# hou-yz/MVDeTr

Hardware: AMD Instinct MI355X
Metric: multiview frames/s (7-cam Wildtrack) + MSDeformAttn HBM GB/s vs roofline (higher is better)
Workload: dtype f32

## Files before the change

include/mvdetr_ops.h:

```cpp
#ifndef MVDETR_OPS_H
#define MVDETR_OPS_H

#include <stdint.h>

#ifdef __cplusplus
extern "C" {
#endif

#define MVDETR_OPS_ABI_VERSION 18

int mvdetr_ops_abi_version(void);

int mvdetr_msda_forward_f32(void *stream, const float *value, const int64_t *spatial_shapes,
                            const int64_t *level_start_index, const float *sampling_loc,
                            const float *attn_weight, int batch, int spatial_size, int num_heads,
                            int channels, int num_levels, int num_query, int num_point, float *out);
int mvdetr_msda_forward_f64(void *stream, const double *value, const int64_t *spatial_shapes,
                            const int64_t *level_start_index, const double *sampling_loc,
                            const double *attn_weight, int batch, int spatial_size, int num_heads,
                            int channels, int num_levels, int num_query, int num_point, double *out);

int mvdetr_msda_forward_f16(void *stream, const uint16_t *value, const int64_t *spatial_shapes,
                            const int64_t *level_start_index, const uint16_t *sampling_loc,
                            const uint16_t *attn_weight, int batch, int spatial_size, int num_heads, int channels,
// ... 120 lines not shown
                               const float *beta, float eps, int n, int h, int w, int channels, float *y);
int mvdetr_bn_act_f16(void *stream, const uint16_t *x, const float *mean, const float *var, const float *gamma,
                      const float *beta, float eps, const uint16_t *res, const float *res_mean, const float *res_var,
                      const float *res_gamma, const float *res_beta, float res_eps, int64_t rows, int channels, int relu,
                      uint16_t *y);
int mvdetr_bn_act_bf16(void *stream, const uint16_t *x, const float *mean, const float *var, const float *gamma,
                       const float *beta, float eps, const uint16_t *res, const float *res_mean, const float *res_var,
                       const float *res_gamma, const float *res_beta, float res_eps, int64_t rows, int channels, int relu,
                       uint16_t *y);
int mvdetr_bn_relu_maxpool_f16(void *stream, const uint16_t *x, const float *mean, const float *var, const float *gamma,
                               const float *beta, float eps, int n, int h, int w, int channels, uint16_t *y);
int mvdetr_bn_relu_maxpool_bf16(void *stream, const uint16_t *x, const float *mean, const float *var, const float *gamma,
                                const float *beta, float eps, int n, int h, int w, int channels, uint16_t *y);
const char *mvdetr_trunk_last_kernel(void);
int64_t mvdetr_trunk_launch_count(void);

int mvdetr_winograd_weights_f32(const float *w, int C, int K, float *U, void *stream);
int mvdetr_conv3x3_winograd_f32(const float *x, const float *U, float *y, int N, int H, int W, int C, int K, int dilation,
                                void *stream);
int mvdetr_conv3x3_winograd_bn_act_f32(const float *x, const float *U, float *y, int N, int H, int W, int C, int K,
                                       int dilation, const float *mean, const float *var, const float *gamma,
                                       const float *beta, float eps, const float *res, const float *res_mean,
                                       const float *res_var, const float *res_gamma, const float *res_beta, float res_eps,
                                       int relu, void *stream);
const char *mvdetr_winograd_last_kernel(void);
const char *mvdetr_winograd_last_epilogue(void);
int64_t mvdetr_winograd_launch_count(void);
int mvdetr_winograd_set_max_workgroups(int n);
int mvdetr_winograd_set_variant(int variant);
int mvdetr_winograd_last_variant(void);
int mvdetr_winograd_set_tail(int mode);
int mvdetr_winograd_last_tail_units(void);
int mvdetr_winograd_plan(int N, int H, int W, int C, int K, int dilation, int workgroups, int64_t *out);

int mvdetr_winograd_weights_dgrad_f32(const float *w, int C, int K, float *Ut, void *stream);
int mvdetr_conv3x3_winograd_wgrad_f32(const float *x, const float *gy, float *gw, int N, int H, int W, int C, int K, int dilation,
                                      void *workspace, int64_t workspace_bytes, void *stream);
int64_t mvdetr_winograd_wgrad_workspace_bytes(int N, int H, int W, int C, int K, int dilation, int workgroups);
int mvdetr_winograd_wgrad_plan(int N, int H, int W, int C, int K, int dilation, int workgroups, int64_t *out);
int mvdetr_winograd_set_wgrad_splits(int n);
int mvdetr_winograd_last_wgrad_splits(void);

const char *mvdetr_msda_last_forward_impl(void);
const char *mvdetr_msda_last_forward_kernel(void);
const char *mvdetr_msda_last_backward_route(void);

int mvdetr_msda_last_forward_resources(int *num_regs, int *scratch_bytes_per_lane, int *static_lds_bytes);

const char *mvdetr_warp_last_kernel(void);

int mvdetr_warp_release_scratch(void);

int mvdetr_msda_set_forward_impl(int impl);

int mvdetr_msda_set_backward_deterministic(int on);
int mvdetr_msda_get_backward_deterministic(void);

int mvdetr_msda_release_scratch(void);

int mvdetr_transpose_f32(void *stream, const float *src, int n, int rows, int cols, float *dst);
int mvdetr_transpose_f64(void *stream, const double *src, int n, int rows, int cols, double *dst);

int mvdetr_deform_conv2d_forward_f32(void *stream, const float *input, const float *offset, const float *weight,
                                     const float *bias, int batch, int in_channels, int in_h, int in_w, int out_channels,
                                     int kernel_h, int kernel_w, int stride_h, int stride_w, int pad_h, int pad_w, int dil_h,
                                     int dil_w, int offset_groups, int input_nhwc, float *out);
// ... 233 lines not shown
```

mvdetr_amd/_lib.py:

```python
from __future__ import annotations

import ctypes
import functools
import os
import subprocess

import torch

_HERE = os.path.dirname(os.path.abspath(__file__))
CSRC = os.path.join(_HERE, "csrc")
LIB_PATH = os.environ.get("MVDETR_OPS_LIB") or os.path.join(CSRC, "libmvdetr_ops.so")
ABI_VERSION = 18

_vp, _i = ctypes.c_void_p, ctypes.c_int
_MSDA_FWD = [_vp] * 6 + [_i] * 7 + [_vp]
_MSDA_BWD = [_vp] * 7 + [_i] * 7 + [_vp] * 3
_WARP = [_vp] * 3 + [_i] * 7 + [_vp]
_MSDA_FWD_HOST = [_vp] * 5 + [_i] * 7 + [_vp]
_MSDA_BWD_HOST = [_vp] * 6 + [_i] * 7 + [_vp] * 3
_WARP_HOST = [_vp] * 2 + [_i] * 8 + [_vp]
_MSDA_FUSED = [_vp] * 5 + [ctypes.c_int64] + [_vp] * 2 + [_i] * 10 + [_vp]
_MSDA_FUSED_HALF = [_vp] * 5 + [ctypes.c_int64, _vp] + [_i] * 7 + [_vp]
_MSDA_FUSED_LEVELS = [_vp] * 5 + [ctypes.c_int64] + [_vp] * 2 + [_i] * 12 + [_vp]
_DC_FWD = [_vp] * 5 + [_i] * 15 + [_vp]
# ... 48 lines not shown
    "mvdetr_msda_forward_fused_bf16": (_MSDA_FUSED_HALF, _i),
    "mvdetr_msda_fused_levels_supported": ([_i] * 9, _i),
    "mvdetr_msda_forward_fused_levels_f32": (_MSDA_FUSED_LEVELS, _i),
    "mvdetr_msda_fused_train_supported": ([_i] * 7, _i),
    "mvdetr_msda_forward_fused_train_f32": ([_vp] * 5 + [ctypes.c_int64, _vp] + [_i] * 7 + [_vp, _vp], _i),
    "mvdetr_msda_backward_fused_f32": ([_vp] * 6 + [ctypes.c_int64, _vp, _i, _vp, _vp] + [_i] * 6 + [_vp, _vp], _i),
    "mvdetr_msda_backward_f32": (_MSDA_BWD, _i),
    "mvdetr_msda_backward_f64": (_MSDA_BWD, _i),
    "mvdetr_add_layernorm_f32": ([_vp] * 5 + [ctypes.c_int64, _i, ctypes.c_float, _vp], _i),
    "mvdetr_add_layernorm_add_f32": ([_vp] * 6 + [ctypes.c_int64, ctypes.c_int64, _i, ctypes.c_float, _vp, _vp], _i),
    "mvdetr_add_layernorm_add_f16": ([_vp] * 6 + [ctypes.c_int64, ctypes.c_int64, _i, ctypes.c_float, _vp, _vp], _i),
    "mvdetr_add_layernorm_add_bf16": ([_vp] * 6 + [ctypes.c_int64, ctypes.c_int64, _i, ctypes.c_float, _vp, _vp], _i),
    "mvdetr_add_layernorm_last_kernel": ([], ctypes.c_char_p),
    "mvdetr_bn_act_f32": ([_vp] * 6 + [ctypes.c_float] + [_vp] * 5 + [ctypes.c_float, ctypes.c_int64, _i, _i, _vp], _i),
    "mvdetr_bn_relu_maxpool_f32": ([_vp] * 6 + [ctypes.c_float] + [_i] * 4 + [_vp], _i),
    "mvdetr_bn_act_f16": ([_vp] * 6 + [ctypes.c_float] + [_vp] * 5 + [ctypes.c_float, ctypes.c_int64, _i, _i, _vp], _i),
    "mvdetr_bn_act_bf16": ([_vp] * 6 + [ctypes.c_float] + [_vp] * 5 + [ctypes.c_float, ctypes.c_int64, _i, _i, _vp], _i),
    "mvdetr_bn_relu_maxpool_f16": ([_vp] * 6 + [ctypes.c_float] + [_i] * 4 + [_vp], _i),
    "mvdetr_bn_relu_maxpool_bf16": ([_vp] * 6 + [ctypes.c_float] + [_i] * 4 + [_vp], _i),
    "mvdetr_trunk_last_kernel": ([], ctypes.c_char_p),
    "mvdetr_trunk_launch_count": ([], ctypes.c_int64),
    "mvdetr_winograd_weights_f32": ([_vp, _i, _i, _vp, _vp], _i),
    "mvdetr_conv3x3_winograd_f32": ([_vp] * 3 + [_i] * 6 + [_vp], _i),
    "mvdetr_conv3x3_winograd_bn_act_f32": ([_vp] * 3 + [_i] * 6 + [_vp] * 4 + [ctypes.c_float] + [_vp] * 5
                                           + [ctypes.c_float, _i, _vp], _i),
    "mvdetr_winograd_last_kernel": ([], ctypes.c_char_p),
    "mvdetr_winograd_last_epilogue": ([], ctypes.c_char_p),
    "mvdetr_winograd_launch_count": ([], ctypes.c_int64),
    "mvdetr_winograd_set_max_workgroups": ([_i], _i),
    "mvdetr_winograd_set_tail": ([_i], _i),
    "mvdetr_winograd_set_variant": ([_i], _i),
    "mvdetr_winograd_last_variant": ([], _i),
    "mvdetr_winograd_last_tail_units": ([], _i),
    "mvdetr_winograd_plan": ([_i] * 7 + [_vp], _i),
    "mvdetr_winograd_weights_dgrad_f32": ([_vp, _i, _i, _vp, _vp], _i),
    "mvdetr_conv3x3_winograd_wgrad_f32": ([_vp] * 3 + [_i] * 6 + [_vp, ctypes.c_int64, _vp], _i),
    "mvdetr_winograd_wgrad_workspace_bytes": ([_i] * 7, ctypes.c_int64),
    "mvdetr_winograd_wgrad_plan": ([_i] * 7 + [_vp], _i),
    "mvdetr_winograd_set_wgrad_splits": ([_i], _i),
    "mvdetr_winograd_last_wgrad_splits": ([], _i),
    "mvdetr_warp_perspective_forward_f32": (_WARP, _i),
    "mvdetr_warp_perspective_forward_f64": (_WARP, _i),
    "mvdetr_warp_perspective_forward_f16": (_WARP, _i),
    "mvdetr_warp_perspective_forward_bf16": (_WARP, _i),
    "mvdetr_warp_perspective_backward_f32": (_WARP, _i),
    "mvdetr_warp_perspective_backward_f64": (_WARP, _i),
    "mvdetr_warp_perspective_backward_tagged_f32": ([_vp] * 3 + [_i] * 7 + [ctypes.c_uint64, _vp], _i),
    "mvdetr_warp_perspective_backward_tagged_f64": ([_vp] * 3 + [_i] * 7 + [ctypes.c_uint64, _vp], _i),
    "mvdetr_warp_backward_plan_bytes": ([_i] * 7, ctypes.c_int64),
    "mvdetr_warp_backward_plan_f32": ([_vp, _vp] + [_i] * 6 + [_vp], _i),
    "mvdetr_warp_backward_plan_f64": ([_vp, _vp] + [_i] * 6 + [_vp], _i),
    "mvdetr_warp_perspective_backward_planned_f32": ([_vp] * 4 + [_i] * 7 + [_vp], _i),
    "mvdetr_warp_perspective_backward_planned_f64": ([_vp] * 4 + [_i] * 7 + [_vp], _i),
    "mvdetr_transpose_f32": ([_vp, _vp, _i, _i, _i, _vp], _i),
    "mvdetr_transpose_f64": ([_vp, _vp, _i, _i, _i, _vp], _i),
    "mvdetr_msda_forward_host_f32": (_MSDA_FWD_HOST, _i),
    "mvdetr_msda_forward_host_f64": (_MSDA_FWD_HOST, _i),
    "mvdetr_msda_backward_host_f32": (_MSDA_BWD_HOST, _i),
    "mvdetr_msda_backward_host_f64": (_MSDA_BWD_HOST, _i),
    "mvdetr_warp_perspective_forward_host_f32": (_WARP_HOST, _i),
    "mvdetr_warp_perspective_forward_host_f64": (_WARP_HOST, _i),
    "mvdetr_warp_perspective_backward_host_f32": (_WARP_HOST, _i),
    "mvdetr_warp_perspective_backward_host_f64": (_WARP_HOST, _i),
    "mvdetr_deform_conv2d_last_kernel": ([], ctypes.c_char_p),
    "mvdetr_deform_conv2d_route_kind": ([_i] * 18, _i),
    "mvdetr_deform_conv2d_forward_f32": (_DC_FWD, _i),
# ... 140 lines not shown
```

mvdetr_amd/csrc/conv_winograd.hip:

```cpp
#include "bn_epilogue.h"
#include "common.h"
#include "conv_winograd.h"
#include "../../include/mvdetr_ops.h"

#include <atomic>
#include <type_traits>

namespace mvdetr {

std::atomic<const char *> g_winograd_last_kernel{"none"};
static std::atomic<const char *> g_winograd_last_epilogue{"none"};
std::atomic<int64_t> g_winograd_launches{0};
std::atomic<int> g_winograd_max_workgroups{0};
static std::atomic<int> g_winograd_tail{1};
static std::atomic<int> g_winograd_last_tail_units{0};
static std::atomic<int> g_winograd_variant{0};
static std::atomic<int> g_winograd_last_variant{0};

namespace wino {

constexpr int CC = 8;
constexpr int VCOLS = TILES + 8;
constexpr int VROW = VCOLS * 4;
constexpr int V_FLOATS = CC * 4 * VROW;
constexpr int U_FLOATS = 16 * CC * KB;
constexpr int BUF_FLOATS = U_FLOATS + V_FLOATS;
constexpr int TINFO_SLOTS = 4;
constexpr int LDS_BYTES = 2 * BUF_FLOATS * 4 + TINFO_SLOTS * TILES * 16;

constexpr unsigned Y_NONE = 0xFFFFFFFFu;

using f32x16 = __attribute__((ext_vector_type(16))) float;
using f32x4 = __attribute__((ext_vector_type(4))) float;

typedef __attribute__((address_space(3))) void lds_void;

struct Epilogue {
    BnVectors bn, bn2;
    const float *res;
};

template <int MODE, bool RELU>
__global__ __launch_bounds__(256) void conv3x3_winograd_f32(const float *__restrict__ x, const float *__restrict__ U,
                                                            float *__restrict__ y, const Shape s, const Epilogue ep)
{
    extern __shared__ __attribute__((aligned(16))) float lds[];
    using u32x4 = __attribute__((ext_vector_type(4))) unsigned;
    u32x4 *const tinfo = reinterpret_cast<u32x4 *>(lds + 2 * BUF_FLOATS);

    const int tid = threadIdx.x, lane = tid & 63;
// ... 461 lines not shown
        const u32x4 dsc = ti[16 * (b >> 2) + (b & 3)];
#pragma unroll
        for (int e = 0; e < 4; ++e) {
            o4[b][e] = __builtin_elementwise_add_sat(dsc[e], (unsigned)kcol * 4u);
            if (MODE >= 2) q4[b][e] = __builtin_bit_cast(float, __builtin_amdgcn_raw_buffer_load_b32(rrsrc, (int)o4[b][e], 0, 0));
        }
    }
#pragma unroll
    for (int b = 0; b < 8; ++b) {
        const int h = b >> 2, r = b & 3;
        float s0[4], s1[4];
#pragma unroll
        for (int nu = 0; nu < 4; ++nu) {
            s0[nu] = acc[nu][h][r] + acc[4 + nu][h][r] + acc[8 + nu][h][r];
            s1[nu] = acc[4 + nu][h][r] - acc[8 + nu][h][r] - acc[12 + nu][h][r];
        }
        float y00 = s0[0] + s0[1] + s0[2], y01 = s0[1] - s0[2] - s0[3];
        float y10 = s1[0] + s1[1] + s1[2], y11 = s1[1] - s1[2] - s1[3];
        if (MODE >= 1) {
            constexpr int RES = MODE - 1;
            y00 = bn_finish<RES, RELU>(bn_apply(y00, bs, bt), RES ? q4[b][0] : 0.f, bs2);
            y01 = bn_finish<RES, RELU>(bn_apply(y01, bs, bt), RES ? q4[b][1] : 0.f, bs2);
            y10 = bn_finish<RES, RELU>(bn_apply(y10, bs, bt), RES ? q4[b][2] : 0.f, bs2);
            y11 = bn_finish<RES, RELU>(bn_apply(y11, bs, bt), RES ? q4[b][3] : 0.f, bs2);
        }
        const float y4[4] = {y00, y01, y10, y11};
#pragma unroll
        for (int e = 0; e < 4; ++e)
            __builtin_amdgcn_raw_buffer_store_b32(__builtin_bit_cast(unsigned, y4[e]), yrsrc, (int)o4[b][e], 0, 0);
    }
    asm volatile("s_waitcnt vmcnt(0)" ::: "memory");
}

template <int MODE, bool RELU>
__global__ __launch_bounds__(512) void conv3x3_winograd_w16x2_f32(const float *__restrict__ x, const float *__restrict__ U,
                                                                  float *__restrict__ y, const Shape s, const Epilogue ep)
{
    extern __shared__ __attribute__((aligned(16))) float lds[];
    using u32x4 = __attribute__((ext_vector_type(4))) unsigned;
    u32x4 *const tinfo = reinterpret_cast<u32x4 *>(lds + 2 * BUF_FLOATS);

    const int tid = threadIdx.x, lane = tid & 63;
    const int wave = __builtin_amdgcn_readfirstlane(tid >> 6);
    const int C = s.C, K = s.K, d = s.d, H = s.H, W = s.W;
    const int chunks = C / CC;
    const unsigned G = gridDim.x;

    const int ltile = tid >> 3, lc = tid & 7;
    unsigned off[16];
    __amdgpu_buffer_rsrc_t xrsrc;
    __amdgpu_buffer_rsrc_t ursrc;
    struct Place { int kb, X, Y, n; };
    auto next_unit = [&](Place &p) {
        p.kb += s.gr;
        const bool carry = p.kb >= s.kblocks;
        p.kb -= carry ? s.kblocks : 0;
        tile_step(s, carry, p.X, p.Y, p.n);
        return carry;
    };
    Place sp, cpl;
    sp.kb = (int)(blockIdx.x % (unsigned)s.kblocks);
    tile_grid(s, blockIdx.x / (unsigned)s.kblocks * TILES, sp.X, sp.Y, sp.n);
    cpl = sp;
    int lX, lY, ln;
    tile_grid(s, blockIdx.x / (unsigned)s.kblocks * TILES + ltile, lX, lY, ln);
    auto enter_unit = [&](int slot) {
        const int n0 = sp.n;
        xrsrc = __builtin_amdgcn_make_buffer_rsrc(const_cast<float *>(x + (size_t)n0 * H * W * C), 0, (int)X_RANGE, 0x00020000);
        ursrc = __builtin_amdgcn_make_buffer_rsrc(const_cast<float *>(U + sp.kb * KB), 0,
                                                  (int)(((unsigned)(16 * C) * K - sp.kb * KB) * 4u), 0x00020000);
        int y0, x0;
        tile_pixel(s, lX, lY, y0, x0);
        const bool tvalid = ln < s.N;
        const unsigned pix = ((unsigned)(ln - n0) * H + y0) * W + x0;
        const unsigned base = (pix * C + lc) * 4u, cstep = (unsigned)d * C * 4u, rstep = cstep * W;
        bool oky[4], okx[4];
// ... 69 lines not shown
    f32x4 acc[16][2];
    float fa[2][2][8], fb[2][8];
    auto read_piece = [&](const float *buf, int hs, int q) {
        const int st = hs >> 1, half = hs & 1;
        if ((q & 2) == 0) {
            const int xl = q >> 2, h = q & 1;
            const f32x4 v = *reinterpret_cast<const f32x4 *>(buf + a_off + (16 * st + 2 * half + xl) * VROW + (16 * h + 4 * st) * 4);
#pragma unroll
            for (int nu = 0; nu < 4; ++nu) fa[half][h][4 * xl + nu] = v[nu];
        } else {
            const int pl = 4 * (q >> 2) + 2 * (q & 1), p = 8 * half + pl;
            fb[half][pl] = buf[b_off + (p * CC + 4 * st) * KB];
            fb[half][pl + 1] = buf[b_off + ((p + 1) * CC + 4 * st) * KB];
        }
    };
    auto mfma = [&](int hs, int m, auto first) {
        const int half = hs & 1, pl = m >> 1, h = m & 1, p = 8 * half + pl;
        if (decltype(first)::value) acc[p][h] = __builtin_amdgcn_mfma_f32_16x16x4f32(fa[half][h][pl], fb[half][pl], f32x4{}, 0, 0, 0);
        else acc[p][h] = __builtin_amdgcn_mfma_f32_16x16x4f32(fa[half][h][pl], fb[half][pl], acc[p][h], 0, 0, 0);
    };

    {
#pragma unroll
        for (int q = 0; q < 16; ++q) load_x(0, q);
#pragma unroll
        for (int r = 0; r < 4; ++r) load_u(0, lds, r);
#pragma unroll
        for (int u = 0; u < 16; ++u) xform_piece(lds, u);
        asm volatile("s_waitcnt vmcnt(0)" ::: "memory");
        __syncthreads();
        advance();
#pragma unroll
        for (int q = 0; q < 16; ++q) load_x(sc * CC, q);
#pragma unroll
        for (int r = 0; r < 4; ++r) load_u(sc * CC, lds + BUF_FLOATS, r);
#pragma unroll
        for (int q = 0; q < 8; ++q) read_piece(lds, 0, q);
    }

    const int kcol = wq * 16 + (lane & 15);
    float bs = 1.f, bt = 0.f, bs2 = 0.f;
    int kb_folded = -1;
    unsigned cu = blockIdx.x;
    int cslot = 0, par = 0;
    auto chunk = [&](auto first) {
        advance();
        float *const cur = lds + par * BUF_FLOATS;
        float *const nxt = lds + (par ^ 1) * BUF_FLOATS;
        __builtin_amdgcn_sched_barrier(0);
#pragma unroll
        for (int m = 0; m < 16; ++m) {
            mfma(0, m, first);
            if (m < 8) read_piece(cur, 1, m);
            __builtin_amdgcn_sched_barrier(0);
        }
#pragma unroll
        for (int m = 0; m < 16; ++m) {
            mfma(1, m, first);
            if (m < 8) read_piece(cur, 2, m);
            else xform_piece(nxt, m - 8);
            __builtin_amdgcn_sched_barrier(0);
        }
#pragma unroll
        for (int m = 0; m < 16; ++m) {
            mfma(2, m, std::false_type{});
            if (m < 8) read_piece(cur, 3, m);
            else xform_piece(nxt, m);
            __builtin_amdgcn_sched_barrier(0);
        }
        asm volatile("s_waitcnt vmcnt(0)" ::: "memory");
        __syncthreads();
#pragma unroll
        for (int m = 0; m < 16; ++m) {
            mfma(3, m, std::false_type{});
            if (m < 8) {
                load_x(sc * CC, 2 * m);
                load_x(sc * CC, 2 * m + 1);
            } else {
                read_piece(nxt, 0, m - 8);
                if (m < 12) load_u(sc * CC, cur, m - 8);
            }
            __builtin_amdgcn_sched_barrier(0);
        }
        par ^= 1;
    };
    do {
        chunk(std::true_type{});
        if (chunks > 1) {
            int ch = 1;
            do chunk(std::false_type{});
            while (++ch < chunks);
        }

        const int kb = cpl.kb, n0 = cpl.n;
        const unsigned long long left = ((unsigned long long)(s.N - n0) * H * W * K - (unsigned)(kb * KB)) * 4ull;
        const int yrange = (int)(left < X_RANGE ? (unsigned)left : X_RANGE);
        const __amdgpu_buffer_rsrc_t yrsrc =
            __builtin_amdgcn_make_buffer_rsrc(y + (size_t)n0 * H * W * K + kb * KB, 0, yrange, 0x00020000);
        const u32x4 *const ti = tinfo + cslot * TILES + th * 32 + 4 * (lane >> 4);
        auto offsets = [&](int b, unsigned (&o4)[4]) {
            const u32x4 dsc = ti[16 * (b >> 2) + (b & 3)];
#pragma unroll
            for (int e = 0; e < 4; ++e) o4[e] = __builtin_elementwise_add_sat(dsc[e], (unsigned)kcol * 4u);
        };
        if (MODE >= 1 && kb != kb_folded) {
            bn_fold1(ep.bn, kb * KB + kcol, bs, bt);
            if (MODE == 3) {
                float bt2;
                bn_fold1(ep.bn2, kb * KB + kcol, bs2, bt2);
                bt = bt + bt2;
            }
            kb_folded = kb;
        }
        float q[2][4][4];
        __amdgpu_buffer_rsrc_t rrsrc;
        if (MODE >= 2)
            rrsrc = __builtin_amdgcn_make_buffer_rsrc(const_cast<float *>(ep.res + (size_t)n0 * H * W * K + kb * KB), 0, yrange,
                                                      0x00020000);
        auto load_res = [&](int h) {
#pragma unroll
            for (int rr = 0; rr < 4; ++rr) {
                unsigned o4[4];
                offsets(4 * h + rr, o4);
#pragma unroll
                for (int e = 0; e < 4; ++e)
                    q[h][rr][e] = __builtin_bit_cast(float, __builtin_amdgcn_raw_buffer_load_b32(rrsrc, (int)o4[e], 0, 0));
            }
        };
        if (MODE >= 2) {
            load_res(0);
            __builtin_amdgcn_sched_barrier(0);
        }
        asm volatile("s_nop 15\n\ts_nop 3");
#pragma unroll
        for (int b = 0; b < 8; ++b) {
            const int h = b >> 2, r = b & 3;
            if (MODE >= 2 && b == 0) {
                load_res(1);
                __builtin_amdgcn_sched_barrier(0);
            }
            unsigned o4[4];
            offsets(b, o4);
            float m[16];
#pragma unroll
            for (int p = 0; p < 16; ++p) asm volatile("v_accvgpr_read_b32 %0, %1" : "=v"(m[p]) : "a"(acc[p][h][r]));
            float s0[4], s1[4];
#pragma unroll
            for (int nu = 0; nu < 4; ++nu) {
                s0[nu] = m[nu] + m[4 + nu] + m[8 + nu];
                s1[nu] = m[4 + nu] - m[8 + nu] - m[12 + nu];
            }
            float y00 = s0[0] + s0[1] + s0[2], y01 = s0[1] - s0[2] - s0[3];
            float y10 = s1[0] + s1[1] + s1[2], y11 = s1[1] - s1[2] - s1[3];
            if (MODE >= 1) {
                constexpr int RES = MODE - 1;
                const float *const qr = q[h][r];
                y00 = bn_finish<RES, RELU>(bn_apply(y00, bs, bt), RES ? qr[0] : 0.f, bs2);
                y01 = bn_finish<RES, RELU>(bn_apply(y01, bs, bt), RES ? qr[1] : 0.f, bs2);
                y10 = bn_finish<RES, RELU>(bn_apply(y10, bs, bt), RES ? qr[2] : 0.f, bs2);
                y11 = bn_finish<RES, RELU>(bn_apply(y11, bs, bt), RES ? qr[3] : 0.f, bs2);
            }
            const float y4[4] = {y00, y01, y10, y11};
#pragma unroll
            for (int e = 0; e < 4; ++e)
                __builtin_amdgcn_raw_buffer_store_b32(__builtin_bit_cast(unsigned, y4[e]), yrsrc, (int)o4[e], 0, 0);
#pragma unroll
            for (int p = 0; p < 16; ++p) asm volatile("" : "+a"(acc[p][0]), "+a"(acc[p][1]));
            __builtin_amdgcn_sched_barrier(0);
        }
        cu += G;
        next_unit(cpl);
        cslot = (cslot + 1) & (TINFO_SLOTS - 1);
    } while (cu < s.units);
    asm volatile("s_waitcnt vmcnt(0)" ::: "memory");
}

__global__ __launch_bounds__(256) void winograd_weights_f32(const float *__restrict__ w, int C, int K, float *__restrict__ U)
{
    const int64_t i = (int64_t)blockIdx.x * 256 + threadIdx.x;
    if (i >= (int64_t)C * K) return;
    const int k = (int)(i % K), c = (int)(i / K);
    const float *g = w + ((size_t)k * C + c) * 9;
    double t[4][3];
#pragma unroll
    for (int j = 0; j < 3; ++j) {
        const double g0 = g[j], g1 = g[3 + j], g2 = g[6 + j];
        t[0][j] = g0;
        t[1][j] = 0.5 * (g0 + g1 + g2);
        t[2][j] = 0.5 * (g0 - g1 + g2);
        t[3][j] = g2;
    }
#pragma unroll
    for (int xi = 0; xi < 4; ++xi) {
        const double u[4] = {t[xi][0], 0.5 * (t[xi][0] + t[xi][1] + t[xi][2]), 0.5 * (t[xi][0] - t[xi][1] + t[xi][2]), t[xi][2]};
#pragma unroll
        for (int nu = 0; nu < 4; ++nu) U[((size_t)(4 * xi + nu) * C + c) * K + k] = (float)u[nu];
    }
}

template <int MODE, bool RELU>
static int launch(hipStream_t st, unsigned blocks, const float *x, const float *U, float *y, const Shape &s, const Epilogue &ep,
                  int variant, unsigned tail_units)
{
    static PerDevice<int> lds_attr;
    const int rc = lds_attr.get([] {
        const void *const kernels[3] = {reinterpret_cast<const void *>(conv3x3_winograd_f32<MODE, RELU>),
                                        reinterpret_cast<const void *>(conv3x3_winograd_w16x2_f32<MODE, RELU>),
                                        reinterpret_cast<const void *>(conv3x3_winograd_w16_f32<MODE, RELU>)};
        for (int i = 0; i < 3; ++i) {
            const int a = (int)hipFuncSetAttribute(kernels[i], hipFuncAttributeMaxDynamicSharedMemorySize, i < 2 ? LDS_BYTES : w16::LDS_BYTES);
            if (a != 0) return a;
        }
        return 0;
    });
    if (rc != 0) return rc;
    if (variant == 2)
        hipLaunchKernelGGL((conv3x3_winograd_w16x2_f32<MODE, RELU>), dim3(blocks), dim3(512), LDS_BYTES, st, x, U, y, s, ep);
    else
        hipLaunchKernelGGL((conv3x3_winograd_f32<MODE, RELU>), dim3(blocks), dim3(256), LDS_BYTES, st, x, U, y, s, ep);
    if (tail_units)
        hipLaunchKernelGGL((conv3x3_winograd_w16_f32<MODE, RELU>), dim3(2 * tail_units), dim3(256), w16::LDS_BYTES, st, x, U, y, s,
                           ep, s.units);
    return 0;
}

static const char *const kEpilogueNames[4][2] = {
    {"none", "none"}, {"bn", "bn_relu"}, {"bn_add", "bn_add_relu"}, {"bn_bn_add", "bn_bn_add_relu"}};

static bool bn_ok(const BnVectors &b)
{
    return b.mean && b.var && aligned(b.mean, 4) && aligned(b.var, 4) && aligned(b.gamma, 4) && aligned(b.beta, 4);
}

static bool tail_family(int C, int K, int d)
{
    static const int table[][3] = {{64, 64, 1}, {128, 128, 1}, {128, 256, 1}, {256, 256, 1}, {256, 256, 2}, {512, 512, 1}};
    for (const auto &f : table)
        if (f[0] == C && f[1] == K && f[2] == d) return true;
    return false;
}

static bool variant2_family(int C, int K, int d)
{
    static const int table[][3] = {{64, 64, 1},  {128, 128, 1}, {128, 256, 1}, {256, 256, 1},
                                   {256, 256, 2}, {256, 512, 2}, {512, 512, 1}, {512, 512, 4}};
    for (const auto &f : table)
        if (f[0] == C && f[1] == K && f[2] == d) return true;
    return false;
}

struct Plan {
    unsigned units, G, R, rem, half_units;
    int variant;
};

static Plan make_plan(const Shape &s, int cus)
{
    Plan p;
    p.units = s.units;
    const int cap = g_winograd_max_workgroups.load();
    p.G = s.units < (unsigned)cus ? s.units : (unsigned)cus;
    if (cap > 0 && p.G > (unsigned)cap) p.G = (unsigned)cap;
    p.R = s.units / p.G;
    p.rem = s.units % p.G;
    const int tail = g_winograd_tail.load();
    const bool on = p.rem > 0 && (tail == 2 || (tail == 1 && 2 * p.rem <= p.G && tail_family(s.C, s.K, s.d)));
    p.half_units = on ? 2 * p.rem : 0;
    const int v = g_winograd_variant.load();
    p.variant = v ? v : variant2_family(s.C, s.K, s.d) ? 2 : 1;
    return p;
}

static int conv_entry(const float *x, const float *U, float *y, int N, int H, int W, int C, int K, int dilation, int mode,
                      bool relu, const Epilogue &ep, void *stream)
{
    if (!x || !U || !y || x == y || N < 0 || H <= 0 || W <= 0 || C <= 0 || K <= 0) return (int)hipErrorInvalidValue;
    if (mode >= 1 && !bn_ok(ep.bn)) return (int)hipErrorInvalidValue;
    if (mode == 3 && !bn_ok(ep.bn2)) return (int)hipErrorInvalidValue;
    if (C % 8 != 0 || K % 64 != 0 || !(dilation == 1 || dilation == 2 || dilation == 4) || !aligned(x, 16) ||
        !aligned(U, 16) || !aligned(y, 16) || (mode >= 2 && !aligned(ep.res, 16)))
        return (int)hipErrorNotSupported;
    if ((256 + 2 * (int64_t)H * W) * (C > K ? C : K) >= (int64_t)1 << 30) return (int)hipErrorNotSupported;
    if ((int64_t)C * K >= (int64_t)1 << 26) return (int)hipErrorNotSupported;
    if (mode >= 2) {
        const uintptr_t r0 = reinterpret_cast<uintptr_t>(ep.res), y0 = reinterpret_cast<uintptr_t>(y);
        const uintptr_t bytes = (uintptr_t)N * H * W * K * 4;
        if (r0 < y0 + bytes && y0 < r0 + bytes) return (int)hipErrorInvalidValue;
    }
    if (N == 0) return 0;
    Shape s;
    if (!tile_shape(s, N, H, W, C, K, dilation)) return (int)hipErrorNotSupported;
    hipStream_t st = reinterpret_cast<hipStream_t>(stream);
    static PerDevice<int> cus_of;
    const int cus = cus_of.get([] {
        int dev = 0, n = 256;
        if (hipGetDevice(&dev) != hipSuccess || hipDeviceGetAttribute(&n, hipDeviceAttributeMultiprocessorCount, dev) != hipSuccess || n <= 0)
            n = 256;
        return n;
    });
    const Plan pl = make_plan(s, cus);
    const unsigned nb = pl.G;
    if (pl.half_units) s.units = pl.R * pl.G;
    s.gr = (int)(nb % (unsigned)s.kblocks);
    const auto stride = [&](int64_t tile_blocks, int &dX, int &dY, int &dn) {
        const int64_t t = tile_blocks * TILES, r = t / s.TX;
        dX = (int)(t % s.TX);
        dY = (int)(r % s.TY);
        dn = (int)(r / s.TY);
    };
    stride(nb / (unsigned)s.kblocks, s.dX0, s.dY0, s.dn0);
    stride(nb / (unsigned)s.kblocks + 1, s.dX1, s.dY1, s.dn1);
    const unsigned tu = pl.half_units / 2;
    int rc;
    if (mode == 0) rc = launch<0, false>(st, nb, x, U, y, s, ep, pl.variant, tu);
    else if (mode == 1) rc = relu ? launch<1, true>(st, nb, x, U, y, s, ep, pl.variant, tu) : launch<1, false>(st, nb, x, U, y, s, ep, pl.variant, tu);
    else if (mode == 2) rc = relu ? launch<2, true>(st, nb, x, U, y, s, ep, pl.variant, tu) : launch<2, false>(st, nb, x, U, y, s, ep, pl.variant, tu);
    else rc = relu ? launch<3, true>(st, nb, x, U, y, s, ep, pl.variant, tu) : launch<3, false>(st, nb, x, U, y, s, ep, pl.variant, tu);
    if (rc != 0) return rc;
    g_winograd_last_tail_units = (int)tu;
    g_winograd_last_variant = pl.variant;
    g_winograd_last_kernel = "conv3x3_winograd_f32";
    g_winograd_last_epilogue = kEpilogueNames[mode][mode && relu ? 1 : 0];
    g_winograd_launches.fetch_add(1);
    return (int)hipGetLastError();
}

}
}

extern "C" int mvdetr_winograd_weights_f32(const float *w, int C, int K, float *U, void *stream)
{
    using namespace mvdetr;
    if (!w || !U || C <= 0 || K <= 0) return (int)hipErrorInvalidValue;
    if (C % 8 != 0 || K % 64 != 0 || !aligned(w, 4) || !aligned(U, 16) || (int64_t)C * K > (int64_t)1 << 26)
        return (int)hipErrorNotSupported;
    hipLaunchKernelGGL(wino::winograd_weights_f32, dim3((unsigned)(((int64_t)C * K + 255) / 256)), dim3(256), 0,
                       reinterpret_cast<hipStream_t>(stream), w, C, K, U);
    g_winograd_last_kernel = "winograd_weights_f32";
    g_winograd_launches.fetch_add(1);
    return (int)hipGetLastError();
}

extern "C" int mvdetr_conv3x3_winograd_f32(const float *x, const float *U, float *y, int N, int H, int W, int C, int K,
                                           int dilation, void *stream)
{
    return mvdetr::wino::conv_entry(x, U, y, N, H, W, C, K, dilation, 0, false, mvdetr::wino::Epilogue{}, stream);
}

extern "C" int mvdetr_conv3x3_winograd_bn_act_f32(const float *x, const float *U, float *y, int N, int H, int W, int C, int K,
                                                  int dilation, const float *mean, const float *var, const float *gamma,
                                                  const float *beta, float eps, const float *res, const float *res_mean,
                                                  const float *res_var, const float *res_gamma, const float *res_beta,
                                                  float res_eps, int relu, void *stream)
{
    using namespace mvdetr;
    const bool res_bn = res_mean || res_var || res_gamma || res_beta;
    if (res_bn && !res) return (int)hipErrorInvalidValue;
    const wino::Epilogue ep{BnVectors{mean, var, gamma, beta, eps}, BnVectors{res_mean, res_var, res_gamma, res_beta, res_eps}, res};
    return wino::conv_entry(x, U, y, N, H, W, C, K, dilation, !res ? 1 : res_bn ? 3 : 2, relu != 0, ep, stream);
}

extern "C" const char *mvdetr_winograd_last_kernel(void) { return mvdetr::g_winograd_last_kernel.load(); }

extern "C" const char *mvdetr_winograd_last_epilogue(void) { return mvdetr::g_winograd_last_epilogue.load(); }

extern "C" int64_t mvdetr_winograd_launch_count(void) { return mvdetr::g_winograd_launches.load(); }

extern "C" int mvdetr_winograd_set_max_workgroups(int n) { return mvdetr::g_winograd_max_workgroups.exchange(n > 0 ? n : 0); }

extern "C" int mvdetr_winograd_set_tail(int mode) { return mvdetr::g_winograd_tail.exchange(mode == 0 || mode == 2 ? mode : 1); }

extern "C" int mvdetr_winograd_set_variant(int v) { return mvdetr::g_winograd_variant.exchange(v == 1 || v == 2 ? v : 0); }

extern "C" int mvdetr_winograd_last_variant(void) { return mvdetr::g_winograd_last_variant.load(); }

extern "C" int mvdetr_winograd_last_tail_units(void) { return mvdetr::g_winograd_last_tail_units.load(); }

extern "C" int mvdetr_winograd_plan(int N, int H, int W, int C, int K, int dilation, int workgroups, int64_t *out)
{
    using namespace mvdetr;
    if (!out || N <= 0 || H <= 0 || W <= 0 || C <= 0 || K <= 0 || workgroups <= 0) return (int)hipErrorInvalidValue;
    wino::Shape s;
    if (C % 8 != 0 || K % 64 != 0 || !(dilation == 1 || dilation == 2 || dilation == 4) ||
        !wino::tile_shape(s, N, H, W, C, K, dilation))
        return (int)hipErrorNotSupported;
    const wino::Plan p = wino::make_plan(s, workgroups);
    out[0] = p.units; out[1] = p.G; out[2] = p.R; out[3] = p.rem; out[4] = p.half_units; out[5] = p.variant;
    return 0;
}
```

mvdetr_amd/ops/conv_winograd.py:

```python
from __future__ import annotations

import os
import weakref

import torch
from torch import nn

from .. import _lib
from . import trunk_epilogue

_enabled = os.environ.get("MVDETR_TRUNK_WINOGRAD", "1") != "0"
_epilogue = os.environ.get("MVDETR_WINOGRAD_EPILOGUE", "1") != "0"
_train_enabled = os.environ.get("MVDETR_TRUNK_WINOGRAD_TRAIN", "1") != "0"

G = ((1.0, 0.0, 0.0), (0.5, 0.5, 0.5), (0.5, -0.5, 0.5), (0.0, 0.0, 1.0))
BT = ((1.0, 0.0, -1.0, 0.0), (0.0, 1.0, 1.0, 0.0), (0.0, -1.0, 1.0, 0.0), (0.0, 1.0, 0.0, -1.0))
AT = ((1.0, 1.0, 1.0, 0.0), (0.0, 1.0, -1.0, -1.0))

FAMILIES: dict = {(128, 256): (1,), (256, 256): (1, 2), (256, 512): (2,), (512, 512): (1, 4)}
DILATIONS = (1, 2, 4)

MIN_PIXELS = 8192
_min_pixels = MIN_PIXELS

# ... 40 lines not shown
    prev, _narrow_min_pixels = _narrow_min_pixels, int(pixels)
    return prev


def last_kernel() -> str:
    return _lib.lib().mvdetr_winograd_last_kernel().decode()


def last_epilogue() -> str:
    return _lib.lib().mvdetr_winograd_last_epilogue().decode()


def launch_count() -> int:
    return int(_lib.lib().mvdetr_winograd_launch_count())


def set_winograd_max_workgroups(n: int) -> int:
    return int(_lib.lib().mvdetr_winograd_set_max_workgroups(int(n)))


TAIL_FAMILIES = ((64, 64, 1), (128, 128, 1), (128, 256, 1), (256, 256, 1), (256, 256, 2), (512, 512, 1))


def set_winograd_tail(mode: int) -> int:
    return int(_lib.lib().mvdetr_winograd_set_tail(int(mode)))


def set_winograd_variant(variant: int) -> int:
    return int(_lib.lib().mvdetr_winograd_set_variant(int(variant)))


def last_variant() -> int:
    return int(_lib.lib().mvdetr_winograd_last_variant())


def last_tail_units() -> int:
    return int(_lib.lib().mvdetr_winograd_last_tail_units())


def plan(N: int, H: int, W: int, C: int, K: int, dilation: int, workgroups: int) -> dict:
    import ctypes
    out = (ctypes.c_int64 * 6)()
    _lib.check(_lib.lib().mvdetr_winograd_plan(N, H, W, C, K, dilation, workgroups, ctypes.cast(out, ctypes.c_void_p)),
               "winograd_plan")
    return dict(zip(("units", "G", "R", "rem", "half_units", "variant"), (int(v) for v in out)))


def _on_device(t) -> bool:
    return t.is_cuda


def _two(v, want) -> bool:
    return v == want or tuple(v) == (want, want)


def _kernel_ok(x, conv) -> bool:
    if not (isinstance(x, torch.Tensor) and x.dim() == 4 and x.dtype == torch.float32 and _on_device(x) and x.numel() > 0
            and x.is_contiguous(memory_format=torch.channels_last) and x.data_ptr() % 16 == 0):
        return False
    if type(conv) is not nn.Conv2d:
        return False
    d = conv.dilation[0]
    if not (_two(conv.kernel_size, 3) and _two(conv.stride, 1) and conv.groups == 1 and conv.bias is None
            and conv.padding_mode == "zeros" and d in DILATIONS and _two(conv.dilation, d)
            and not isinstance(conv.padding, str) and _two(conv.padding, d)):
        return False
# ... 273 lines not shown
```

Measured before the change: 76.32.

## Add wave-role schedule to w16x2 Winograd conv with staggered load/transform phases

Adds a second schedule for the w16x2 Winograd conv kernel. In it, waves 4-7 run at raised priority with a different interleaving of U loads, x loads and input transforms across the four MFMA phases, while waves 0-3 keep the original order. The schedule is on by default for a listed set of channel and dilation families. The intent is to desynchronise the two wave groups so memory loads and LDS transforms overlap MFMA work better. It risks register pressure and hazards from the reordered phases.

```diff
diff --git a/include/mvdetr_ops.h b/include/mvdetr_ops.h
--- a/include/mvdetr_ops.h
+++ b/include/mvdetr_ops.h
@@ -176,6 +176,9 @@
 int mvdetr_winograd_set_tail(int mode);
 int mvdetr_winograd_last_tail_units(void);
 int mvdetr_winograd_plan(int N, int H, int W, int C, int K, int dilation, int workgroups, int64_t *out);
+int mvdetr_winograd_set_schedule(int schedule);
+int mvdetr_winograd_last_schedule(void);
+int mvdetr_winograd_schedule_of(int C, int K, int dilation);
 
 int mvdetr_winograd_weights_dgrad_f32(const float *w, int C, int K, float *Ut, void *stream);
 int mvdetr_conv3x3_winograd_wgrad_f32(const float *x, const float *gy, float *gw, int N, int H, int W, int C, int K, int dilation,
diff --git a/mvdetr_amd/_lib.py b/mvdetr_amd/_lib.py
--- a/mvdetr_amd/_lib.py
+++ b/mvdetr_amd/_lib.py
@@ -104,6 +104,9 @@
     "mvdetr_winograd_set_variant": ([_i], _i),
     "mvdetr_winograd_last_variant": ([], _i),
     "mvdetr_winograd_last_tail_units": ([], _i),
+    "mvdetr_winograd_set_schedule": ([_i], _i),
+    "mvdetr_winograd_last_schedule": ([], _i),
+    "mvdetr_winograd_schedule_of": ([_i] * 3, _i),
     "mvdetr_winograd_plan": ([_i] * 7 + [_vp], _i),
     "mvdetr_winograd_weights_dgrad_f32": ([_vp, _i, _i, _vp, _vp], _i),
     "mvdetr_conv3x3_winograd_wgrad_f32": ([_vp] * 3 + [_i] * 6 + [_vp, ctypes.c_int64, _vp], _i),
diff --git a/mvdetr_amd/csrc/conv_winograd.hip b/mvdetr_amd/csrc/conv_winograd.hip
--- a/mvdetr_amd/csrc/conv_winograd.hip
+++ b/mvdetr_amd/csrc/conv_winograd.hip
@@ -16,6 +16,8 @@
 static std::atomic<int> g_winograd_last_tail_units{0};
 static std::atomic<int> g_winograd_variant{0};
 static std::atomic<int> g_winograd_last_variant{0};
+static std::atomic<int> g_winograd_schedule{0};
+static std::atomic<int> g_winograd_last_schedule{0};
 
 namespace wino {
 
@@ -543,16 +545,18 @@
     asm volatile("s_waitcnt vmcnt(0)" ::: "memory");
 }
 
-template <int MODE, bool RELU>
-__global__ __launch_bounds__(512) void conv3x3_winograd_w16x2_f32(const float *__restrict__ x, const float *__restrict__ U,
-                                                                  float *__restrict__ y, const Shape s, const Epilogue ep)
+template <int MODE, bool RELU, int DEAL, bool ROLES>
+__device__ __forceinline__ void conv3x3_winograd_w16x2_deal(const float *__restrict__ x, const float *__restrict__ U,
+                                                            float *__restrict__ y, const Shape &s, const Epilogue &ep,
+                                                            const int wave)
 {
     extern __shared__ __attribute__((aligned(16))) float lds[];
     using u32x4 = __attribute__((ext_vector_type(4))) unsigned;
     u32x4 *const tinfo = reinterpret_cast<u32x4 *>(lds + 2 * BUF_FLOATS);
 
-    const int tid = threadIdx.x, lane = tid & 63;
-    const int wave = __builtin_amdgcn_readfirstlane(tid >> 6);
+    int lane = threadIdx.x & 63;
+    if (ROLES) asm volatile("v_mbcnt_lo_u32_b32 %0, -1, 0\n\tv_mbcnt_hi_u32_b32 %0, -1, %0 ; deal %1" : "=v"(lane) : "n"(DEAL));
+    const int tid = wave * 64 + lane;
     const int C = s.C, K = s.K, d = s.d, H = s.H, W = s.W;
     const int chunks = C / CC;
     const unsigned G = gridDim.x;
@@ -688,8 +692,13 @@
         advance();
 #pragma unroll
         for (int q = 0; q < 16; ++q) load_x(sc * CC, q);
-#pragma unroll
-        for (int r = 0; r < 4; ++r) load_u(sc * CC, lds + BUF_FLOATS, r);
+        if (DEAL == 1) {
+#pragma unroll
+            for (int u = 0; u < 8; ++u) xform_piece(lds + BUF_FLOATS, u);
+        } else {
+#pragma unroll
+            for (int r = 0; r < 4; ++r) load_u(sc * CC, lds + BUF_FLOATS, r);
+        }
 #pragma unroll
         for (int q = 0; q < 8; ++q) read_piece(lds, 0, q);
     }
@@ -699,8 +708,9 @@
     int kb_folded = -1;
     unsigned cu = blockIdx.x;
     int cslot = 0, par = 0;
-    auto chunk = [&](auto first) {
-        advance();
+    auto chunk = [&](auto first, auto deal) {
+        constexpr int D = decltype(deal)::value;
+        if (D == 0) advance();
         float *const cur = lds + par * BUF_FLOATS;
         float *const nxt = lds + (par ^ 1) * BUF_FLOATS;
         __builtin_amdgcn_sched_barrier(0);
@@ -708,20 +718,32 @@
         for (int m = 0; m < 16; ++m) {
             mfma(0, m, first);
             if (m < 8) read_piece(cur, 1, m);
+            if (D == 1 && m < 4) load_u(sc * CC, nxt, m);
+            if (D == 1 && m >= 8) xform_piece(nxt, m);
+            __builtin_amdgcn_sched_barrier(0);
+        }
+        if (D != 0) {
+            advance();
             __builtin_amdgcn_sched_barrier(0);
         }
 #pragma unroll
         for (int m = 0; m < 16; ++m) {
             mfma(1, m, first);
-            if (m < 8) read_piece(cur, 2, m);
-            else xform_piece(nxt, m - 8);
+            if (m < 8) {
+                read_piece(cur, 2, m);
+            } else if (D == 1) {
+                load_x(sc * CC, 2 * (m - 8));
+                load_x(sc * CC, 2 * (m - 8) + 1);
+            } else {
+                xform_piece(nxt, m - 8);
+            }
             __builtin_amdgcn_sched_barrier(0);
         }
 #pragma unroll
         for (int m = 0; m < 16; ++m) {
             mfma(2, m, std::false_type{});
             if (m < 8) read_piece(cur, 3, m);
-            else xform_piece(nxt, m);
+            else if (D == 0) xform_piece(nxt, m);
             __builtin_amdgcn_sched_barrier(0);
         }
         asm volatile("s_waitcnt vmcnt(0)" ::: "memory");
@@ -729,106 +751,131 @@
 #pragma unroll
         for (int m = 0; m < 16; ++m) {
             mfma(3, m, std::false_type{});
-            if (m < 8) {
-                load_x(sc * CC, 2 * m);
-                load_x(sc * CC, 2 * m + 1);
-            } else {
+            if (D == 0) {
+                if (m < 8) {
+                    load_x(sc * CC, 2 * m);
+                    load_x(sc * CC, 2 * m + 1);
+                } else {
+                    read_piece(nxt, 0, m - 8);
+                    if (m < 12) load_u(sc * CC, cur, m - 8);
+                }
+            } else if (m >= 8) {
                 read_piece(nxt, 0, m - 8);
-                if (m < 12) load_u(sc * CC, cur, m - 8);
+                xform_piece(cur, m - 8);
             }
             __builtin_amdgcn_sched_barrier(0);
         }
         par ^= 1;
     };
-    do {
-        chunk(std::true_type{});
+    auto unit_chunks = [&](auto deal) {
+        chunk(std::true_type{}, deal);
         if (chunks > 1) {
             int ch = 1;
-            do chunk(std::false_type{});
+            do chunk(std::false_type{}, deal);
             while (++ch < chunks);
         }
-
-        const int kb = cpl.kb, n0 = cpl.n;
-        const unsigned long long left = ((unsigned long long)(s.N - n0) * H * W * K - (unsigned)(kb * KB)) * 4ull;
-        const int yrange = (int)(left < X_RANGE ? (unsigned)left : X_RANGE);
-        const __amdgpu_buffer_rsrc_t yrsrc =
-            __builtin_amdgcn_make_buffer_rsrc(y + (size_t)n0 * H * W * K + kb * KB, 0, yrange, 0x00020000);
-        const u32x4 *const ti = tinfo + cslot * TILES + th * 32 + 4 * (lane >> 4);
-        auto offsets = [&](int b, unsigned (&o4)[4]) {
-            const u32x4 dsc = ti[16 * (b >> 2) + (b & 3)];
-#pragma unroll
-            for (int e = 0; e < 4; ++e) o4[e] = __builtin_elementwise_add_sat(dsc[e], (unsigned)kcol * 4u);
-        };
-        if (MODE >= 1 && kb != kb_folded) {
-            bn_fold1(ep.bn, kb * KB + kcol, bs, bt);
-            if (MODE == 3) {
-                float bt2;
-                bn_fold1(ep.bn2, kb * KB + kcol, bs2, bt2);
-                bt = bt + bt2;
-            }
-            kb_folded = kb;
-        }
-        float q[2][4][4];
-        __amdgpu_buffer_rsrc_t rrsrc;
-        if (MODE >= 2)
-            rrsrc = __builtin_amdgcn_make_buffer_rsrc(const_cast<float *>(ep.res + (size_t)n0 * H * W * K + kb * KB), 0, yrange,
-                                                      0x00020000);
-        auto load_res = [&](int h) {
-#pragma unroll
-            for (int rr = 0; rr < 4; ++rr) {
+    };
+    auto units = [&](auto deal) {
+        do {
+            unit_chunks(deal);
+
+            const int kb = cpl.kb, n0 = cpl.n;
+            const unsigned long long left = ((unsigned long long)(s.N - n0) * H * W * K - (unsigned)(kb * KB)) * 4ull;
+            const int yrange = (int)(left < X_RANGE ? (unsigned)left : X_RANGE);
+            const __amdgpu_buffer_rsrc_t yrsrc =
+                __builtin_amdgcn_make_buffer_rsrc(y + (size_t)n0 * H * W * K + kb * KB, 0, yrange, 0x00020000);
+            const u32x4 *const ti = tinfo + cslot * TILES + th * 32 + 4 * (lane >> 4);
+            auto offsets = [&](int b, unsigned (&o4)[4]) {
+                const u32x4 dsc = ti[16 * (b >> 2) + (b & 3)];
+#pragma unroll
+                for (int e = 0; e < 4; ++e) o4[e] = __builtin_elementwise_add_sat(dsc[e], (unsigned)kcol * 4u);
+            };
+            if (MODE >= 1 && kb != kb_folded) {
+                bn_fold1(ep.bn, kb * KB + kcol, bs, bt);
+                if (MODE == 3) {
+                    float bt2;
+                    bn_fold1(ep.bn2, kb * KB + kcol, bs2, bt2);
+                    bt = bt + bt2;
+                }
+                kb_folded = kb;
+            }
+            constexpr int RES1_AT = ROLES && MODE == 3 ? 2 : 0;
+            float q[2][4][4];
+            __amdgpu_buffer_rsrc_t rrsrc;
+            if (MODE >= 2)
+                rrsrc = __builtin_amdgcn_make_buffer_rsrc(const_cast<float *>(ep.res + (size_t)n0 * H * W * K + kb * KB), 0, yrange,
+                                                          0x00020000);
+            auto load_res = [&](int h) {
+#pragma unroll
+                for (int rr = 0; rr < 4; ++rr) {
+                    unsigned o4[4];
+                    offsets(4 * h + rr, o4);
+#pragma unroll
+                    for (int e = 0; e < 4; ++e)
+                        q[h][rr][e] = __builtin_bit_cast(float, __builtin_amdgcn_raw_buffer_load_b32(rrsrc, (int)o4[e], 0, 0));
+                }
+            };
+            if (MODE >= 2) {
+                load_res(0);
+                __builtin_amdgcn_sched_barrier(0);
+            }
+            asm volatile("s_nop 15\n\ts_nop 3");
+#pragma unroll
+            for (int b = 0; b < 8; ++b) {
+                const int h = b >> 2, r = b & 3;
+                if (MODE >= 2 && b == RES1_AT) {
+                    load_res(1);
+                    __builtin_amdgcn_sched_barrier(0);
+                }
                 unsigned o4[4];
-                offsets(4 * h + rr, o4);
+                offsets(b, o4);
+                float m[16];
+#pragma unroll
+                for (int p = 0; p < 16; ++p) asm volatile("v_accvgpr_read_b32 %0, %1" : "=v"(m[p]) : "a"(acc[p][h][r]));
+                float s0[4], s1[4];
+#pragma unroll
+                for (int nu = 0; nu < 4; ++nu) {
+                    s0[nu] = m[nu] + m[4 + nu] + m[8 + nu];
+                    s1[nu] = m[4 + nu] - m[8 + nu] - m[12 + nu];
+                }
+                float y00 = s0[0] + s0[1] + s0[2], y01 = s0[1] - s0[2] - s0[3];
+                float y10 = s1[0] + s1[1] + s1[2], y11 = s1[1] - s1[2] - s1[3];
+                if (MODE >= 1) {
+                    constexpr int RES = MODE - 1;
+                    const float *const qr = q[h][r];
+                    y00 = bn_finish<RES, RELU>(bn_apply(y00, bs, bt), RES ? qr[0] : 0.f, bs2);
+                    y01 = bn_finish<RES, RELU>(bn_apply(y01, bs, bt), RES ? qr[1] : 0.f, bs2);
+                    y10 = bn_finish<RES, RELU>(bn_apply(y10, bs, bt), RES ? qr[2] : 0.f, bs2);
+                    y11 = bn_finish<RES, RELU>(bn_apply(y11, bs, bt), RES ? qr[3] : 0.f, bs2);
+                }
+                const float y4[4] = {y00, y01, y10, y11};
 #pragma unroll
                 for (int e = 0; e < 4; ++e)
-                    q[h][rr][e] = __builtin_bit_cast(float, __builtin_amdgcn_raw_buffer_load_b32(rrsrc, (int)o4[e], 0, 0));
-            }
-        };
-        if (MODE >= 2) {
-            load_res(0);
-            __builtin_amdgcn_sched_barrier(0);
-        }
-        asm volatile("s_nop 15\n\ts_nop 3");
-#pragma unroll
-        for (int b = 0; b < 8; ++b) {
-            const int h = b >> 2, r = b & 3;
-            if (MODE >= 2 && b == 0) {
-                load_res(1);
+                    __builtin_amdgcn_raw_buffer_store_b32(__builtin_bit_cast(unsigned, y4[e]), yrsrc, (int)o4[e], 0, 0);
+#pragma unroll
+                for (int p = 0; p < 16; ++p) asm volatile("" : "+a"(acc[p][0]), "+a"(acc[p][1]));
                 __builtin_amdgcn_sched_barrier(0);
             }
-            unsigned o4[4];
-            offsets(b, o4);
-            float m[16];
-#pragma unroll
-            for (int p = 0; p < 16; ++p) asm volatile("v_accvgpr_read_b32 %0, %1" : "=v"(m[p]) : "a"(acc[p][h][r]));
-            float s0[4], s1[4];
-#pragma unroll
-            for (int nu = 0; nu < 4; ++nu) {
-                s0[nu] = m[nu] + m[4 + nu] + m[8 + nu];
-                s1[nu] = m[4 + nu] - m[8 + nu] - m[12 + nu];
-            }
-            float y00 = s0[0] + s0[1] + s0[2], y01 = s0[1] - s0[2] - s0[3];
-            float y10 = s1[0] + s1[1] + s1[2], y11 = s1[1] - s1[2] - s1[3];
-            if (MODE >= 1) {
-                constexpr int RES = MODE - 1;
-                const float *const qr = q[h][r];
-                y00 = bn_finish<RES, RELU>(bn_apply(y00, bs, bt), RES ? qr[0] : 0.f, bs2);
-                y01 = bn_finish<RES, RELU>(bn_apply(y01, bs, bt), RES ? qr[1] : 0.f, bs2);
-                y10 = bn_finish<RES, RELU>(bn_apply(y10, bs, bt), RES ? qr[2] : 0.f, bs2);
-                y11 = bn_finish<RES, RELU>(bn_apply(y11, bs, bt), RES ? qr[3] : 0.f, bs2);
-            }
-            const float y4[4] = {y00, y01, y10, y11};
-#pragma unroll
-            for (int e = 0; e < 4; ++e)
-                __builtin_amdgcn_raw_buffer_store_b32(__builtin_bit_cast(unsigned, y4[e]), yrsrc, (int)o4[e], 0, 0);
-#pragma unroll
-            for (int p = 0; p < 16; ++p) asm volatile("" : "+a"(acc[p][0]), "+a"(acc[p][1]));
-            __builtin_amdgcn_sched_barrier(0);
-        }
-        cu += G;
-        next_unit(cpl);
-        cslot = (cslot + 1) & (TINFO_SLOTS - 1);
-    } while (cu < s.units);
+            cu += G;
+            next_unit(cpl);
+            cslot = (cslot + 1) & (TINFO_SLOTS - 1);
+        } while (cu < s.units);
+    };
+    units(std::integral_constant<int, DEAL>{});
     asm volatile("s_waitcnt vmcnt(0)" ::: "memory");
+}
+
+template <int MODE, bool RELU, int SCHED>
+__global__ __launch_bounds__(512) void conv3x3_winograd_w16x2_f32(const float *__restrict__ x, const float *__restrict__ U,
+                                                                  float *__restrict__ y, const Shape s, const Epilogue ep)
+{
+    const int wave = __builtin_amdgcn_readfirstlane(threadIdx.x >> 6);
+    if (SCHED == 2 && wave >= 4) {
+        __builtin_amdgcn_s_setprio(1);
+        conv3x3_winograd_w16x2_deal<MODE, RELU, 1, true>(x, U, y, s, ep, wave);
+    } else {
+        conv3x3_winograd_w16x2_deal<MODE, RELU, 0, SCHED == 2>(x, U, y, s, ep, wave);
+    }
 }
 
 __global__ __launch_bounds__(256) void winograd_weights_f32(const float *__restrict__ w, int C, int K, float *__restrict__ U)
@@ -856,22 +903,25 @@
 
 template <int MODE, bool RELU>
 static int launch(hipStream_t st, unsigned blocks, const float *x, const float *U, float *y, const Shape &s, const Epilogue &ep,
-                  int variant, unsigned tail_units)
+                  int variant, int schedule, unsigned tail_units)
 {
     static PerDevice<int> lds_attr;
     const int rc = lds_attr.get([] {
-        const void *const kernels[3] = {reinterpret_cast<const void *>(conv3x3_winograd_f32<MODE, RELU>),
-                                        reinterpret_cast<const void *>(conv3x3_winograd_w16x2_f32<MODE, RELU>),
-                                        reinterpret_cast<const void *>(conv3x3_winograd_w16_f32<MODE, RELU>)};
-        for (int i = 0; i < 3; ++i) {
-            const int a = (int)hipFuncSetAttribute(kernels[i], hipFuncAttributeMaxDynamicSharedMemorySize, i < 2 ? LDS_BYTES : w16::LDS_BYTES);
+        const void *const kernels[4] = {reinterpret_cast<const void *>(conv3x3_winograd_w16_f32<MODE, RELU>),
+                                        reinterpret_cast<const void *>(conv3x3_winograd_f32<MODE, RELU>),
+                                        reinterpret_cast<const void *>(conv3x3_winograd_w16x2_f32<MODE, RELU, 1>),
+                                        reinterpret_cast<const void *>(conv3x3_winograd_w16x2_f32<MODE, RELU, 2>)};
+        for (int i = 0; i < 4; ++i) {
+            const int a = (int)hipFuncSetAttribute(kernels[i], hipFuncAttributeMaxDynamicSharedMemorySize, i ? LDS_BYTES : w16::LDS_BYTES);
             if (a != 0) return a;
         }
         return 0;
     });
     if (rc != 0) return rc;
-    if (variant == 2)
-        hipLaunchKernelGGL((conv3x3_winograd_w16x2_f32<MODE, RELU>), dim3(blocks), dim3(512), LDS_BYTES, st, x, U, y, s, ep);
+    if (variant == 2 && schedule == 2)
+        hipLaunchKernelGGL((conv3x3_winograd_w16x2_f32<MODE, RELU, 2>), dim3(blocks), dim3(512), LDS_BYTES, st, x, U, y, s, ep);
+    else if (variant == 2)
+        hipLaunchKernelGGL((conv3x3_winograd_w16x2_f32<MODE, RELU, 1>), dim3(blocks), dim3(512), LDS_BYTES, st, x, U, y, s, ep);
     else
         hipLaunchKernelGGL((conv3x3_winograd_f32<MODE, RELU>), dim3(blocks), dim3(256), LDS_BYTES, st, x, U, y, s, ep);
     if (tail_units)
@@ -903,6 +953,20 @@
     for (const auto &f : table)
         if (f[0] == C && f[1] == K && f[2] == d) return true;
     return false;
+}
+
+static bool schedule_family(int C, int K, int d)
+{
+    static const int table[][3] = {{64, 64, 1}, {128, 128, 1}, {256, 256, 1}, {256, 256, 2}, {256, 512, 2}, {512, 512, 1}, {512, 512, 4}};
+    for (const auto &f : table)
+        if (f[0] == C && f[1] == K && f[2] == d) return true;
+    return false;
+}
+
+static int schedule_of(int C, int K, int d)
+{
+    const int v = g_winograd_schedule.load();
+    return v ? v : schedule_family(C, K, d) ? 2 : 1;
 }
 
 struct Plan {
@@ -967,14 +1031,16 @@
     stride(nb / (unsigned)s.kblocks, s.dX0, s.dY0, s.dn0);
     stride(nb / (unsigned)s.kblocks + 1, s.dX1, s.dY1, s.dn1);
     const unsigned tu = pl.half_units / 2;
+    const int sch = pl.variant == 2 ? schedule_of(C, K, dilation) : 1;
     int rc;
-    if (mode == 0) rc = launch<0, false>(st, nb, x, U, y, s, ep, pl.variant, tu);
-    else if (mode == 1) rc = relu ? launch<1, true>(st, nb, x, U, y, s, ep, pl.variant, tu) : launch<1, false>(st, nb, x, U, y, s, ep, pl.variant, tu);
-    else if (mode == 2) rc = relu ? launch<2, true>(st, nb, x, U, y, s, ep, pl.variant, tu) : launch<2, false>(st, nb, x, U, y, s, ep, pl.variant, tu);
-    else rc = relu ? launch<3, true>(st, nb, x, U, y, s, ep, pl.variant, tu) : launch<3, false>(st, nb, x, U, y, s, ep, pl.variant, tu);
+    if (mode == 0) rc = launch<0, false>(st, nb, x, U, y, s, ep, pl.variant, sch, tu);
+    else if (mode == 1) rc = relu ? launch<1, true>(st, nb, x, U, y, s, ep, pl.variant, sch, tu) : launch<1, false>(st, nb, x, U, y, s, ep, pl.variant, sch, tu);
+    else if (mode == 2) rc = relu ? launch<2, true>(st, nb, x, U, y, s, ep, pl.variant, sch, tu) : launch<2, false>(st, nb, x, U, y, s, ep, pl.variant, sch, tu);
+    else rc = relu ? launch<3, true>(st, nb, x, U, y, s, ep, pl.variant, sch, tu) : launch<3, false>(st, nb, x, U, y, s, ep, pl.variant, sch, tu);
     if (rc != 0) return rc;
     g_winograd_last_tail_units = (int)tu;
     g_winograd_last_variant = pl.variant;
+    g_winograd_last_schedule = sch;
     g_winograd_last_kernel = "conv3x3_winograd_f32";
     g_winograd_last_epilogue = kEpilogueNames[mode][mode && relu ? 1 : 0];
     g_winograd_launches.fetch_add(1);
@@ -1030,6 +1096,12 @@
 
 extern "C" int mvdetr_winograd_last_variant(void) { return mvdetr::g_winograd_last_variant.load(); }
 
+extern "C" int mvdetr_winograd_set_schedule(int v) { return mvdetr::g_winograd_schedule.exchange(v == 1 || v == 2 ? v : 0); }
+
+extern "C" int mvdetr_winograd_last_schedule(void) { return mvdetr::g_winograd_last_schedule.load(); }
+
+extern "C" int mvdetr_winograd_schedule_of(int C, int K, int dilation) { return mvdetr::wino::schedule_of(C, K, dilation); }
+
 extern "C" int mvdetr_winograd_last_tail_units(void) { return mvdetr::g_winograd_last_tail_units.load(); }
 
 extern "C" int mvdetr_winograd_plan(int N, int H, int W, int C, int K, int dilation, int workgroups, int64_t *out)
diff --git a/mvdetr_amd/ops/conv_winograd.py b/mvdetr_amd/ops/conv_winograd.py
--- a/mvdetr_amd/ops/conv_winograd.py
+++ b/mvdetr_amd/ops/conv_winograd.py
@@ -96,6 +96,21 @@
 
 def last_variant() -> int:
     return int(_lib.lib().mvdetr_winograd_last_variant())
+
+
+SCHEDULE_FAMILIES = ((64, 64, 1), (128, 128, 1), (256, 256, 1), (256, 256, 2), (256, 512, 2), (512, 512, 1), (512, 512, 4))
+
+
+def set_winograd_schedule(schedule: int) -> int:
+    return int(_lib.lib().mvdetr_winograd_set_schedule(int(schedule)))
+
+
+def last_schedule() -> int:
+    return int(_lib.lib().mvdetr_winograd_last_schedule())
+
+
+def schedule_of(C: int, K: int, dilation: int) -> int:
+    return int(_lib.lib().mvdetr_winograd_schedule_of(int(C), int(K), int(dilation)))
 
 
 def last_tail_units() -> int:
```

Measured after the change: 79.06 (median of 6 runs). +3.6%, better.
